# ignacio-rocco/detectorch

Hardware: AMD Instinct MI355X
Metric: images/sec Mask R-CNN R-50-FPN 1333x800 (region-proposal hot path) (higher is better)
Workload: dtype f32

## Files before the change

### detectorch_amd/csrc/roi_align.hip

```cpp
#include <stdlib.h>

#include <type_traits>

#include "roi_align_common.h"

namespace dtc {

constexpr int kRoiAlignThreads = 256;
constexpr int kMaxTableEntries = 2048;

template <typename TOut>
__device__ __forceinline__ void zero_outputs(TOut* out, int n) {
  for (int o = threadIdx.x; o < n; o += kRoiAlignThreads) out[o] = from_f32<TOut>(0.f);
}

__device__ __forceinline__ void build_axis_tables(AxisEntry* tab, const RoiHead& hd, const dtc_feat_level& L, int ny, int nx,
                                                  int ymul = 1, int xmul = 1) {
  for (int t = threadIdx.x; t < ny + nx; t += kRoiAlignThreads) {
    const bool is_y = t < ny;
    const int u = is_y ? t : t - ny, g = is_y ? hd.gh : hd.gw, mul = is_y ? ymul : xmul;
    AxisEntry e = make_axis(is_y ? hd.sh : hd.sw, is_y ? hd.bin_h : hd.bin_w, u / g, u % g, g, is_y ? L.height : L.width);
    e.lo *= mul; e.hi *= mul;
    tab[t] = e;
  }
// ... 489 lines not shown
  const bool vec = full && ((L.stride_h | L.stride_w | L.stride_n) & 3) == 0 && ((c0 & 3) == 0) &&
                   (reinterpret_cast<uintptr_t>(L.data) & 15) == 0;
  if (4 * q < nc) {
    for (int bin = slot; bin < bins; bin += kRoiAlignThreads / NQ4) {
      const int ph = bin / p.pooled_w, pw = bin - ph * p.pooled_w;
      float a0 = 0.f, a1 = 0.f, a2 = 0.f, a3 = 0.f;
      if (vec && tab_ok && gh == 2 && gw == 2) {
        const AxisEntry x0e = xtab[pw * 2], x1e = xtab[pw * 2 + 1];
        const AxisEntry y0e = ytab[ph * 2], y1e = ytab[ph * 2 + 1];
        float4 t[16];
        t[0] = load4(base + y0e.lo + x0e.lo); t[1] = load4(base + y0e.lo + x0e.hi);
        t[2] = load4(base + y0e.hi + x0e.lo); t[3] = load4(base + y0e.hi + x0e.hi);
        t[4] = load4(base + y0e.lo + x1e.lo); t[5] = load4(base + y0e.lo + x1e.hi);
        t[6] = load4(base + y0e.hi + x1e.lo); t[7] = load4(base + y0e.hi + x1e.hi);
        t[8] = load4(base + y1e.lo + x0e.lo); t[9] = load4(base + y1e.lo + x0e.hi);
        t[10] = load4(base + y1e.hi + x0e.lo); t[11] = load4(base + y1e.hi + x0e.hi);
        t[12] = load4(base + y1e.lo + x1e.lo); t[13] = load4(base + y1e.lo + x1e.hi);
        t[14] = load4(base + y1e.hi + x1e.lo); t[15] = load4(base + y1e.hi + x1e.hi);
#pragma unroll
        for (int sidx = 0; sidx < 4; sidx++) {
          const AxisEntry& y = (sidx < 2) ? y0e : y1e;
          const AxisEntry& x = (sidx & 1) ? x1e : x0e;
          const float w1 = y.h * x.h, w2 = y.h * x.l, w3 = y.l * x.h, w4 = y.l * x.l;
          const float4 v1 = t[sidx * 4], v2 = t[sidx * 4 + 1], v3 = t[sidx * 4 + 2], v4 = t[sidx * 4 + 3];
          a0 += w1 * v1.x + w2 * v2.x + w3 * v3.x + w4 * v4.x;
          a1 += w1 * v1.y + w2 * v2.y + w3 * v3.y + w4 * v4.y;
          a2 += w1 * v1.z + w2 * v2.z + w3 * v3.z + w4 * v4.z;
          a3 += w1 * v1.w + w2 * v2.w + w3 * v3.w + w4 * v4.w;
        }
      } else {
      for (int iy = 0; iy < gh; iy++) {
        const AxisEntry y = tab_ok ? ytab[ph * gh + iy] : [&] { AxisEntry e = make_axis(sh, bin_h, ph, iy, gh, L.height); e.lo *= (int)L.stride_h; e.hi *= (int)L.stride_h; return e; }();
        for (int ix = 0; ix < gw; ix++) {
          const AxisEntry x = tab_ok ? xtab[pw * gw + ix] : [&] { AxisEntry e = make_axis(sw, bin_w, pw, ix, gw, L.width); e.lo *= (int)L.stride_w; e.hi *= (int)L.stride_w; return e; }();
          const float w1 = y.h * x.h, w2 = y.h * x.l, w3 = y.l * x.h, w4 = y.l * x.l;
          float4 v1, v2, v3, v4;
          if (vec) {
            v1 = load4(base + y.lo + x.lo); v2 = load4(base + y.lo + x.hi);
            v3 = load4(base + y.hi + x.lo); v4 = load4(base + y.hi + x.hi);
          } else {
            const TIn* t1 = base + y.lo + x.lo; const TIn* t2 = base + y.lo + x.hi;
            const TIn* t3 = base + y.hi + x.lo; const TIn* t4 = base + y.hi + x.hi;
            const int nv = nc - 4 * q;
            v1 = make_float4(to_f32<TIn>(t1[0]), nv > 1 ? to_f32<TIn>(t1[1]) : 0.f, nv > 2 ? to_f32<TIn>(t1[2]) : 0.f, nv > 3 ? to_f32<TIn>(t1[3]) : 0.f);
            v2 = make_float4(to_f32<TIn>(t2[0]), nv > 1 ? to_f32<TIn>(t2[1]) : 0.f, nv > 2 ? to_f32<TIn>(t2[2]) : 0.f, nv > 3 ? to_f32<TIn>(t2[3]) : 0.f);
            v3 = make_float4(to_f32<TIn>(t3[0]), nv > 1 ? to_f32<TIn>(t3[1]) : 0.f, nv > 2 ? to_f32<TIn>(t3[2]) : 0.f, nv > 3 ? to_f32<TIn>(t3[3]) : 0.f);
            v4 = make_float4(to_f32<TIn>(t4[0]), nv > 1 ? to_f32<TIn>(t4[1]) : 0.f, nv > 2 ? to_f32<TIn>(t4[2]) : 0.f, nv > 3 ? to_f32<TIn>(t4[3]) : 0.f);
          }
          a0 += w1 * v1.x + w2 * v2.x + w3 * v3.x + w4 * v4.x;
          a1 += w1 * v1.y + w2 * v2.y + w3 * v3.y + w4 * v4.y;
          a2 += w1 * v1.z + w2 * v2.z + w3 * v3.z + w4 * v4.z;
          a3 += w1 * v1.w + w2 * v2.w + w3 * v3.w + w4 * v4.w;
        }
      }
      }
      float* so = slab + (4 * q) * bins + bin;
      if (inv_count != 0.f) { so[0] = a0 * inv_count; so[bins] = a1 * inv_count; so[2 * bins] = a2 * inv_count; so[3 * bins] = a3 * inv_count; }
      else { so[0] = fdiv(a0, count); so[bins] = fdiv(a1, count); so[2 * bins] = fdiv(a2, count); so[3 * bins] = fdiv(a3, count); }
    }
  }
  __syncthreads();
  store_slab_vec<TOut, kRoiAlignThreads>(out, slab, nc * bins, tid);
}

const RoiAlignKnobs& roi_align_knobs() {
  static const RoiAlignKnobs knobs = [] {
    RoiAlignKnobs k;
    const auto first_not_0 = [](const char* name, bool dflt) { const char* e = getenv(name); return e ? e[0] != '0' : dflt; };
    const auto is_set = [](const char* name) { return getenv(name) != nullptr; };
    const auto number = [](const char* name, int dflt) { const char* e = getenv(name); return e ? atoi(e) : dflt; };
    const auto in_range = [&](const char* name, int lo, int hi, int dflt) { const int v = number(name, dflt); return v >= lo && v <= hi ? v : dflt; };
    k.tile = first_not_0("DTC_ROIALIGN_TILE", true);
    k.map = first_not_0("DTC_ROIALIGN_MAP", true);
    k.general = is_set("DTC_ROIALIGN_GENERAL");
    k.nhwc_direct = !is_set("DTC_ROIALIGN_NO_NHWC_DIRECT");
    k.nhwc16 = first_not_0("DTC_RA_NHWC16", true);
    k.nhwc_direct32 = first_not_0("DTC_RA_NHWC_DIRECT32", true);
    k.xcd = !is_set("DTC_RA_NO_XCD");
    k.cts64 = !is_set("DTC_RA_NO_CTS64");
    const int cb = number("DTC_RA_TILE_CHBLOCK", 0);
    if (cb >= 4 && (cb & 3) == 0) k.tile_ch_block = cb;
    k.tile_cb_major = number("DTC_RA_TILE_CBMAJOR", 1) != 0;
    k.tile_lds16_kb = in_range("DTC_RA_TILE_LDS16_KB", 36, 156, 0);
    k.map_prep = number("DTC_RA_MAP_PREP", 1) != 0;
    k.map_pitch = first_not_0("DTC_RA_MAP_PITCH", true);
    k.nhwc_lds = number("DTC_RA_NHWC_LDS", 1) != 0;
    k.nhwc_lds_kb = in_range("DTC_RA_NHWC_LDS_KB", 24, 160, 0);
    k.nhwc_pipe = in_range("DTC_RA_NHWC_PIPE", 0, 2, 1);
    k.nhwc_pipe16 = number("DTC_RA_NHWC_PIPE16", 0) != 0;
    k.nhwc_lds_16bit = number("DTC_RA_NHWC_LDS_16BIT", 0) != 0;
    return k;
  }();
  return knobs;
}

constexpr int kLdsKernelBytes = 52 * 1024;

template <typename TIn, typename TOut, int CB>
static int launch_nhwc_cb(const RoiAlignParams& p, hipStream_t stream) {
  const size_t smem = (size_t)kLdsTableFloats * 4 + (size_t)CB * p.pooled_h * p.pooled_w * 4 + 16;
  if (raise_lds_once<roi_align_fwd_nhwc<TIn, TOut, CB>>(160 * 1024) != DTC_OK) return DTC_ELAUNCH;
  const int nct = ceil_div(p.channels, CB);
  hipLaunchKernelGGL((roi_align_fwd_nhwc<TIn, TOut, CB>), dim3((unsigned)p.n_rois * nct), dim3(kRoiAlignThreads), smem, stream, p);
  DTC_CHECK_LAUNCH();
  return DTC_OK;
}

template <typename TIn, typename TOut>
static int launch_nhwc(const RoiAlignParams& p, hipStream_t stream) {
  if (p.n_rois == 0) return DTC_OK;
  if constexpr (sizeof(TIn) == 2) {
    if (p.pooled_h * p.pooled_w > 64 && p.channels % 32 == 0) return launch_nhwc_cb<TIn, TOut, 32>(p, stream);
  }
  return launch_nhwc_cb<TIn, TOut, 64>(p, stream);
}

template <typename TIn, typename TOut>
static int launch_lds(const RoiAlignParams& p, hipStream_t stream) {
  if (p.n_rois == 0) return DTC_OK;
  if (raise_lds_once<roi_align_fwd_lds<TIn, TOut>>(160 * 1024) != DTC_OK) return DTC_ELAUNCH;
  const int nct = ceil_div(p.channels, p.ch_block);
  hipLaunchKernelGGL((roi_align_fwd_lds<TIn, TOut>), dim3((unsigned)p.n_rois * nct), dim3(kRoiAlignThreads), kLdsKernelBytes, stream, p,
                     kLdsKernelBytes / 4);
  DTC_CHECK_LAUNCH();
  return DTC_OK;
}

template <typename TIn, typename TOut>
static int launch_general(const RoiAlignParams& p, hipStream_t stream) {
  if (p.n_rois == 0) return DTC_OK;
  int entries = p.sampling_ratio > 0 ? (p.pooled_h + p.pooled_w) * p.sampling_ratio : kMaxTableEntries;
  if (entries > kMaxTableEntries) entries = kMaxTableEntries;
  size_t smem = (size_t)entries * sizeof(AxisEntry);
  dim3 grid(p.n_rois, ceil_div(p.channels, p.ch_tile));
  hipLaunchKernelGGL((roi_align_fwd_general<TIn, TOut>), grid, dim3(kRoiAlignThreads), smem, stream, p);
  DTC_CHECK_LAUNCH();
  return DTC_OK;
}

enum { kKernNhwc, kKernLds, kKernGeneral };
static int launch_typed(int kind, const RoiAlignParams& p, int in_dtype, int out_dtype, hipStream_t s) {
  return dispatch_io_pair(in_dtype, out_dtype, [&](auto tin, auto tout) {
    typedef tag_type<decltype(tin)> TIn;
    typedef tag_type<decltype(tout)> TOut;
    return kind == kKernNhwc ? launch_nhwc<TIn, TOut>(p, s) : kind == kKernLds ? launch_lds<TIn, TOut>(p, s) : launch_general<TIn, TOut>(p, s);
  });
}

}

static int roi_align_dispatch(const dtc_feat_level* levels, int n_levels, int channels, int in_dtype, const float* rois,
                             int roi_cols, const int32_t* roi_levels, const int32_t* roi_order, const float* roi_desc,
                             int n_rois, int pooled_h, int pooled_w, int sampling_ratio, void* out, int out_dtype,
                             dtc_stream_t stream, void* workspace = nullptr, size_t workspace_bytes = 0) {
  if (!levels || n_levels < 1 || n_levels > DTC_MAX_LEVELS || channels < 1 || n_rois < 0 || pooled_h < 1 ||
      pooled_w < 1 || (roi_cols != 4 && roi_cols != 5) || (n_rois > 0 && ((!rois && !roi_desc) || !out)))
    return DTC_EINVAL;
  const dtc::RoiAlignKnobs& cfg = dtc::roi_align_knobs();
  dtc::RoiAlignParams p;
  for (int i = 0; i < n_levels; i++) {
    if (!levels[i].data || levels[i].height < 1 || levels[i].width < 1) return DTC_EINVAL;
    p.lv[i] = levels[i];
  }
  p.rois = rois; p.roi_levels = roi_levels; p.roi_order = roi_order; p.roi_desc = roi_desc; p.out = out;
  p.n_levels = n_levels; p.channels = channels; p.roi_cols = roi_cols; p.n_rois = n_rois;
  p.pooled_h = pooled_h; p.pooled_w = pooled_w; p.sampling_ratio = sampling_ratio;
// ... 73 lines not shown
```

### detectorch_amd/csrc/roi_align_common.h

```cpp
#pragma once
#include "dtc_common.h"

namespace dtc {

struct RoiAlignParams {
  dtc_feat_level lv[DTC_MAX_LEVELS];
  const float* rois;
  const int32_t* roi_levels;
  const int32_t* roi_order;
  const float* roi_desc;
  void* out;
  int n_levels, channels, roi_cols, n_rois, pooled_h, pooled_w, sampling_ratio, ch_tile;
  int ch_block;
  int cts64;
  int xcd_remap;
  const void* prep = nullptr;
};

constexpr int kXcds = 8;
__device__ __forceinline__ int xcd_work_item(int b, int n, int enabled) {
  if (!enabled || n < 2 * kXcds) return b;
  const int x = b % kXcds, j = b / kXcds;
  const int q = n / kXcds, r = n - q * kXcds;
  return x * q + min(x, r) + j;
// ... 44 lines not shown
    w.d0 = make_float4(b, roi[0], roi[1], roi[2]);
    w.d1 = make_float4(roi[3], (float)lvl, (float)r, 0.f);
  }
  return w;
}

__device__ __forceinline__ RoiHead roi_head_from_raw(const RoiAlignParams& p, const RoiRaw& w) {
  RoiHead h;
  h.b = (int)w.d0.x; h.lvl = (int)w.d1.y; h.r = (int)w.d1.z;
  const float x1 = w.d0.y, y1 = w.d0.z, x2 = w.d0.w, y2 = w.d1.x;
  h.sw = h.sh = 0.f; h.rw = h.rh = 1.f; h.bin_h = h.bin_w = 1.f; h.gh = h.gw = 1; h.count = 1.f; h.inv_count = 1.f;
  if (h.lvl < 0 || h.lvl >= p.n_levels) return h;
  const float s = p.lv[h.lvl].spatial_scale;
  h.sw = x1 * s; h.sh = y1 * s;
  const float ew = x2 * s, eh = y2 * s;
  h.rw = fmaxf(ew - h.sw, 1.f); h.rh = fmaxf(eh - h.sh, 1.f);
  h.bin_h = fdiv(h.rh, (float)p.pooled_h); h.bin_w = fdiv(h.rw, (float)p.pooled_w);
  h.gh = p.sampling_ratio > 0 ? p.sampling_ratio : (int)ceilf(fdiv(h.rh, (float)p.pooled_h));
  h.gw = p.sampling_ratio > 0 ? p.sampling_ratio : (int)ceilf(fdiv(h.rw, (float)p.pooled_w));
  const int gg = h.gh * h.gw;
  h.count = (float)gg;
  h.inv_count = ((gg & (gg - 1)) == 0) ? fdiv(1.f, h.count) : 0.f;
  return h;
}

__device__ __forceinline__ RoiHead load_roi_head(const RoiAlignParams& p, int ri) {
  return roi_head_from_raw(p, load_roi_raw(p, ri));
}

template <typename T> __device__ __forceinline__ f32x2 mul_pair16(uint32_t u, float w);
template <> __device__ __forceinline__ f32x2 mul_pair16<__half>(uint32_t u, float w) {
  f32x2 r;
  asm("v_fma_mix_f32 %0, %2, %3, %4 op_sel:[0,0,0] op_sel_hi:[1,0,0]\n\tv_fma_mix_f32 %1, %2, %3, %4 op_sel:[1,0,0] op_sel_hi:[1,0,0]"
      : "=&v"(r.x), "=&v"(r.y) : "v"(u), "v"(w), "s"(-0.0f));
  return r;
}
template <> __device__ __forceinline__ f32x2 mul_pair16<bf16_t>(uint32_t u, float w) {
  const f32x2 v = {__uint_as_float(u << 16), __uint_as_float(u & 0xffff0000u)};
  return v * w;
}
template <> __device__ __forceinline__ f32x2 mul_pair16<float>(uint32_t, float) { return f32x2{0.f, 0.f}; }

template <typename T> __device__ __forceinline__ void fma_pair16(f32x2& acc, uint32_t u, float w);
template <> __device__ __forceinline__ void fma_pair16<__half>(f32x2& acc, uint32_t u, float w) {
  asm("v_fma_mix_f32 %0, %2, %3, %0 op_sel:[0,0,0] op_sel_hi:[1,0,0]\n\tv_fma_mix_f32 %1, %2, %3, %1 op_sel:[1,0,0] op_sel_hi:[1,0,0]"
      : "+v"(acc.x), "+v"(acc.y) : "v"(u), "v"(w));
}
template <> __device__ __forceinline__ void fma_pair16<bf16_t>(f32x2& acc, uint32_t u, float w) {
  const f32x2 v = {__uint_as_float(u << 16), __uint_as_float(u & 0xffff0000u)};
  const f32x2 w2 = {w, w};
  acc = __builtin_elementwise_fma(v, w2, acc);
}
template <> __device__ __forceinline__ void fma_pair16<float>(f32x2&, uint32_t, float) {}

template <typename T> struct dtype_tag { typedef T type; };
template <typename Tag> using tag_type = typename Tag::type;
template <typename F>
inline int dispatch_io_pair(int in_dtype, int out_dtype, F&& f) {
  if (in_dtype == DTC_F32 && out_dtype == DTC_F32) return f(dtype_tag<float>{}, dtype_tag<float>{});
  if (in_dtype == DTC_F16 && out_dtype == DTC_F32) return f(dtype_tag<__half>{}, dtype_tag<float>{});
  if (in_dtype == DTC_F16 && out_dtype == DTC_F16) return f(dtype_tag<__half>{}, dtype_tag<__half>{});
  if (in_dtype == DTC_F32 && out_dtype == DTC_F16) return f(dtype_tag<float>{}, dtype_tag<__half>{});
  if (in_dtype == DTC_BF16 && out_dtype == DTC_F32) return f(dtype_tag<bf16_t>{}, dtype_tag<float>{});
  if (in_dtype == DTC_BF16 && out_dtype == DTC_BF16) return f(dtype_tag<bf16_t>{}, dtype_tag<bf16_t>{});
  if (in_dtype == DTC_F32 && out_dtype == DTC_BF16) return f(dtype_tag<float>{}, dtype_tag<bf16_t>{});
  return DTC_EUNSUPPORTED;
}
inline bool io_pair_supported(int in_dtype, int out_dtype) {
  return dispatch_io_pair(in_dtype, out_dtype, [](auto, auto) { return (int)DTC_OK; }) == DTC_OK;
}

struct RoiAlignKnobs {
  bool tile = true;
  bool map = true;
  bool general = false;
  bool nhwc_direct = true;
  bool nhwc16 = true;
  bool nhwc_direct32 = true;
  bool xcd = true;
  bool cts64 = true;
  int tile_ch_block = 0;
  int tile_cb_major = 1;
  int tile_lds16_kb = 0;
  bool map_prep = true;
  bool map_pitch = true;
  int nhwc_lds = 1;
  int nhwc_lds_kb = 0;
  int nhwc_pipe = 1;
  int nhwc_pipe16 = 0;
  bool nhwc_lds_16bit = false;
};
const RoiAlignKnobs& roi_align_knobs();

bool roi_align_tile_supported(const RoiAlignParams& p, int in_dtype, int out_dtype);
int launch_roi_align_tile(const RoiAlignParams& p, int in_dtype, int out_dtype, hipStream_t stream);
bool roi_align_map_supported(const RoiAlignParams& p, int in_dtype, int out_dtype);
int launch_roi_align_map(const RoiAlignParams& p, int in_dtype, int out_dtype, hipStream_t stream);
void roi_align_set_exact(int exact);
int roi_align_get_exact();
size_t roi_align_map_workspace_bytes(int n_rois);
int launch_roi_align_map_ws(const RoiAlignParams& p, int in_dtype, int out_dtype, void* workspace, size_t workspace_bytes, hipStream_t stream);

bool roi_align_nhwc_lds_supported(const RoiAlignParams& p, int in_dtype, int out_dtype);
int launch_roi_align_nhwc_lds(const RoiAlignParams& p, int in_dtype, int out_dtype, hipStream_t stream);

bool roi_align_nhwc16_supported(const RoiAlignParams& p, int in_dtype, int out_dtype);
int launch_roi_align_nhwc16(const RoiAlignParams& p, int in_dtype, int out_dtype, hipStream_t stream);

}
```

### detectorch_amd/csrc/roi_align_tile.hip

```cpp

#include <type_traits>

#include "roi_align_common.h"

namespace dtc {

constexpr int kTileMaxK = 32;
constexpr int kTileRoiBytes = 48, kTileGroupBytes = 32;
constexpr int kTileHdrBytes = kTileMaxK * (kTileRoiBytes + kTileGroupBytes) + 16;
template <int NT> struct TileShape;
template <> struct TileShape<256> { static constexpr int kUnits = 8, kWaves = 3, kLdsKB = 52, kWaves16 = 4, kLds16KB = 38; };

struct TileRoi {
  int lvl, b, x0, x1, y0, y1, r, valid;
  float sh, sw, bin_h, bin_w;
};
static_assert(sizeof(TileRoi) == kTileRoiBytes, "TileRoi layout");
struct TileGroup { int first, count, kind, x0, x1, y0, y1, pad; };
enum { kGrpPool = 0, kGrpZero = 1, kGrpAbsent = 2, kGrpGather = 3 };

__device__ __forceinline__ __amdgpu_buffer_rsrc_t make_srd(const void* base) {
  return __builtin_amdgcn_make_buffer_rsrc(const_cast<void*>(base), 0, 0xffffffff, 0x00020000);
}
template <typename TIn> struct Piece4;
template <> struct Piece4<float> {
  typedef float4 Raw;
  static __device__ __forceinline__ Raw raw(__amdgpu_buffer_rsrc_t r, uint32_t voff, uint32_t soff) { return ld(r, voff, soff); }
  static __device__ __forceinline__ float4 ld(__amdgpu_buffer_rsrc_t r, uint32_t voff, uint32_t soff) {
    const u32x4 v = __builtin_amdgcn_raw_buffer_load_b128(r, voff, soff, 0);
    return make_float4(__uint_as_float(v.x), __uint_as_float(v.y), __uint_as_float(v.z), __uint_as_float(v.w));
  }
};
template <> struct Piece4<__half> {
  typedef u32x2 Raw;
  static __device__ __forceinline__ Raw raw(__amdgpu_buffer_rsrc_t r, uint32_t voff, uint32_t soff) { return __builtin_amdgcn_raw_buffer_load_b64(r, voff, soff, 0); }
  static __device__ __forceinline__ float4 ld(__amdgpu_buffer_rsrc_t r, uint32_t voff, uint32_t soff) {
    const u32x2 v = __builtin_amdgcn_raw_buffer_load_b64(r, voff, soff, 0);
    const uint32_t x = v.x, y = v.y;
    const __half2 a = *reinterpret_cast<const __half2*>(&x), b = *reinterpret_cast<const __half2*>(&y);
    return make_float4(__low2float(a), __high2float(a), __low2float(b), __high2float(b));
  }
};
template <> struct Piece4<bf16_t> {
  typedef u32x2 Raw;
  static __device__ __forceinline__ Raw raw(__amdgpu_buffer_rsrc_t r, uint32_t voff, uint32_t soff) { return __builtin_amdgcn_raw_buffer_load_b64(r, voff, soff, 0); }
  static __device__ __forceinline__ float4 ld(__amdgpu_buffer_rsrc_t r, uint32_t voff, uint32_t soff) {
    const u32x2 v = __builtin_amdgcn_raw_buffer_load_b64(r, voff, soff, 0);
    return bf16x4_to_f32(make_uint2(v.x, v.y));
  }
};

__device__ __forceinline__ int uni(int v) { return __builtin_amdgcn_readfirstlane(v); }

#ifdef DTC_TILE_TRACE
constexpr int kTraceSlots = 16;
__device__ unsigned long long g_tile_trace[kTraceSlots * 16384];
struct TileTrace {
  unsigned long long last, acc[kTraceSlots];
  __device__ __forceinline__ void start() { for (int i = 0; i < kTraceSlots; i++) acc[i] = 0; last = __builtin_readcyclecounter(); }
  __device__ __forceinline__ void mark(int i) { const unsigned long long n = __builtin_readcyclecounter(); acc[i] += n - last; last = n; }
};
#define TT_MARK(i) tt.mark(i)
#else
struct TileTrace {};
#define TT_MARK(i) ((void)0)
#endif

template <typename TIn> struct TileLds { typedef float T; static constexpr int kSlot = 16, kShift = 4; };
template <> struct TileLds<__half> { typedef uint16_t T; static constexpr int kSlot = 8, kShift = 3; };
template <> struct TileLds<bf16_t> { typedef uint16_t T; static constexpr int kSlot = 8, kShift = 3; };

template <typename TIn, int NT> struct TileBounds { static constexpr int kWaves = TileShape<NT>::kWaves; };
template <int NT> struct TileBounds<__half, NT> { static constexpr int kWaves = TileShape<NT>::kWaves16; };
template <int NT> struct TileBounds<bf16_t, NT> { static constexpr int kWaves = TileShape<NT>::kWaves16; };

__device__ __forceinline__ int tile_phys(int px) { return px + (px >> 3); }

struct TileItem {
  int a[2][2][4];
  float yl[2], yh[2], xl[2], xh[2];
  bool on;
};

template <typename TOut> __device__ __forceinline__ void store_quad(TOut* d, float4 v);
template <> __device__ __forceinline__ void store_quad<float>(float* d, float4 v) { store_stream16(d, v); }
template <> __device__ __forceinline__ void store_quad<__half>(__half* d, float4 v) {
  const __half2 a = __floats2half2_rn(v.x, v.y), b = __floats2half2_rn(v.z, v.w);
  store_stream8(d, *reinterpret_cast<const uint32_t*>(&a), *reinterpret_cast<const uint32_t*>(&b));
}
template <> __device__ __forceinline__ void store_quad<bf16_t>(bf16_t* d, float4 v) {
  store_stream8(d, (uint32_t)from_f32<bf16_t>(v.x).bits | ((uint32_t)from_f32<bf16_t>(v.y).bits << 16),
                (uint32_t)from_f32<bf16_t>(v.z).bits | ((uint32_t)from_f32<bf16_t>(v.w).bits << 16));
}

enum { kStageScalar = 0, kStageVec = 1, kStageVecUnaligned = 2 };

struct TileGeom {
  int first, count;
  int y0, x0a, ngx, npos;
  int plane;
  int nq_pass;
  int mode;
};

template <typename TIn, typename TOut, int NT, bool FUSED>
__device__ __forceinline__ void tile_passes(const RoiAlignParams& p, const dtc_feat_level& L, const TIn* fbase, int c0, int nc,
                                            int bins, float* slab, typename TileLds<TIn>::T* win, const TileRoi* troi, const TileGeom& g,
                                            const TileItem& it, int rl, int bin, TileTrace& tt) {
  constexpr int NW = NT / 64;
  constexpr int U = TileShape<NT>::kUnits;
  typedef typename TileLds<TIn>::T TL;
  constexpr bool L16 = sizeof(TL) == 2;
  constexpr int SB = TileLds<TIn>::kSlot;
  const int tid = threadIdx.x, lane = tid & 63, wv = tid >> 6, pl = lane & 15, cl = (lane >> 4) & 3;
  const int npos = g.npos, ngx = g.ngx, plane = g.plane, nq_pass = g.nq_pass;
  const int nchunk = (npos + 15) >> 4;
  const int KC = ceil_div(nchunk, NW);
  const float rinv = 1.0f / (float)ngx;
  const int nq_tot = ceil_div(nc, 4);
  const bool vec = g.mode != kStageScalar;
  uint32_t uoff[U];
  int ulds[U];
  const int nu = KC * nq_pass;
  if (vec) {
    const int sh32 = (int)L.stride_h, sc32 = (int)L.stride_c;
    int q = 0, i = 0;
#pragma unroll
    for (int u = 0; u < U; u++) {
      const bool dup = u >= nu;
      const int pos = min((wv + (dup ? 0 : i) * NW) * 16 + pl, npos - 1);
      const int row = (int)(((float)pos + 0.5f) * rinv);
      const int gx = pos - row * ngx;
      const int qq = dup ? 0 : q;
      int col = g.x0a + 4 * gx, sft = 0;
      if (g.mode == kStageVecUnaligned) { sft = max(0, col + 3 - (L.width - 1)); col -= sft; }
      uoff[u] = ((uint32_t)((g.y0 + row) * sh32 + col + (4 * qq + cl) * sc32) * (uint32_t)sizeof(TIn)) | ((uint32_t)sft << 30);
      ulds[u] = qq * plane * 4 + ((4 * pos + (pos >> 1)) << 2) + cl;
      if (++i == KC) { i = 0; q++; }
    }
  }
  const __amdgpu_buffer_rsrc_t srd = make_srd(fbase);
  const uint32_t pass_bytes = (uint32_t)(L.stride_c * (int64_t)sizeof(TIn));
  typename Piece4<TIn>::Raw v[U];
  auto issue = [&](int cs) {
    const uint32_t soff = (uint32_t)cs * pass_bytes;
    if (g.mode == kStageVec) {
#pragma unroll
      for (int u = 0; u < U; u++) v[u] = Piece4<TIn>::raw(srd, uoff[u], soff);
    } else {
#pragma unroll
      for (int u = 0; u < U; u++) v[u] = Piece4<TIn>::raw(srd, uoff[u] & 0x3fffffffu, soff);
    }
  };
  auto commit_as = [&](auto shifted_tag) {
    constexpr bool SHIFTED = decltype(shifted_tag)::value;
    if constexpr (SHIFTED) asm volatile("" ::: "memory");
#pragma unroll
    for (int u = 0; u < U; u++) {
      if constexpr (L16) {
        uint32_t w0 = v[u].x & 0xffffu, w1 = v[u].x >> 16, w2 = v[u].y & 0xffffu, w3 = v[u].y >> 16;
        if constexpr (SHIFTED) {
          const uint32_t sft = uoff[u] >> 30;
          w0 = sft == 0 ? w0 : sft == 1 ? w1 : sft == 2 ? w2 : w3;
          w1 = sft == 0 ? w1 : sft == 1 ? w2 : w3;
          w2 = sft == 0 ? w2 : w3;
        }
        TL* d = win + ulds[u];
        d[0] = (TL)w0; d[4] = (TL)w1; d[8] = (TL)w2; d[12] = (TL)w3;
      } else {
        float4 w = v[u];
        if constexpr (SHIFTED) {
          const uint32_t sft = uoff[u] >> 30;
          w.x = sft == 0 ? w.x : sft == 1 ? w.y : sft == 2 ? w.z : w.w;
          w.y = sft == 0 ? w.y : sft == 1 ? w.z : w.w;
          w.z = sft == 0 ? w.z : w.w;
        }
        TL* d = win + ulds[u];
        d[0] = w.x; d[4] = w.y; d[8] = w.z; d[12] = w.w;
      }
    }
  };
  auto commit = [&]() {
    if (g.mode == kStageVecUnaligned) commit_as(std::true_type{}); else commit_as(std::false_type{});
  };
  auto lds_val = [&](const TIn& x) -> TL {
    if constexpr (L16) return *reinterpret_cast<const uint16_t*>(&x); else return to_f32<TIn>(x);
  };
  auto stage_scalar = [&](int cs) {
#pragma unroll 1
    for (int q = 0; q < nq_pass; q++) {
      const int cq = cs + 4 * q;
      if (cq >= nc) break;
      const int cle = min(cl, nc - 1 - cq);
      const TIn* base = fbase + (int64_t)(cq + cle) * L.stride_c;
#pragma unroll 1
      for (int t = wv; t < nchunk; t += NW) {
        const int pos = min(t * 16 + pl, npos - 1);
        const int row = (int)(((float)pos + 0.5f) * rinv);
        const int gx = pos - row * ngx;
        const int rem = L.width - 1 - (g.x0a + 4 * gx);
        const TIn* s = base + (int64_t)(g.y0 + row) * L.stride_h + (int64_t)(g.x0a + 4 * gx) * L.stride_w;
        TL* d = win + q * plane * 4 + ((4 * pos + (pos >> 1)) << 2) + cl;
        d[0] = lds_val(s[0]);
        d[4] = lds_val(s[(int64_t)min(1, rem) * L.stride_w]);
        d[8] = lds_val(s[(int64_t)min(2, rem) * L.stride_w]);
        d[12] = lds_val(s[(int64_t)min(3, rem) * L.stride_w]);
      }
    }
  };
  const bool quad_ok = ((p.channels | c0) & 3) == 0;
  auto store_slab = [&](int cs, int nq) {
    const int nch = min(4 * nq, nc - cs);
    TOut* out = reinterpret_cast<TOut*>(p.out);
    if (quad_ok && nch == 4 * nq) {
      const int n4 = nq * bins, total = g.count * n4;
      const float r4 = 1.0f / (float)n4;
      const int cs_off = cs * bins;
      for (int idx = tid; idx < total; idx += NT) {
        const int k = (int)(((float)idx + 0.5f) * r4);
        const int e = idx - __mul24(k, n4);
        const float4 val = reinterpret_cast<const float4*>(slab)[idx];
        const uint64_t ob = *reinterpret_cast<const uint64_t*>(&troi[g.first + k].x0);
        store_quad<TOut>(out + (ob + (uint64_t)(uint32_t)(cs_off + 4 * e)), val);
      }
    } else {
      const int per = nch * bins, total = g.count * per;
      for (int idx = tid; idx < total; idx += NT) {
        const int k = idx / per, e = idx - k * per;
        out[((size_t)troi[g.first + k].r * p.channels + c0 + cs) * bins + e] = from_f32<TOut>(slab[k * 4 * nq * bins + e]);
      }
    }
  };

#ifdef DTC_TILE_REPLAY
  {
    uint32_t sink = 0;
    if (DTC_TILE_REPLAY == 1 || DTC_TILE_REPLAY == 4) { if (vec) issue(0); }
    int cs_prev = 0, nq_prev = 0;
#pragma unroll 1
    for (int qs = 0; qs < nq_tot; qs += nq_pass) {
      const int cs = 4 * qs;
      const int nq_cur = min(nq_pass, nq_tot - qs);
      if (DTC_TILE_REPLAY == 1) {
#pragma unroll
        for (int u = 0; u < U; u++) { if constexpr (L16) sink ^= v[u].x ^ v[u].y; else sink ^= __float_as_uint(v[u].x) ^ __float_as_uint(v[u].w); }
        if (vec && qs + nq_pass < nq_tot) issue(cs + 4 * nq_pass);
      } else if (DTC_TILE_REPLAY == 4) {
        if (vec) commit(); else stage_scalar(cs);
        __syncthreads();
        if (vec && qs + nq_pass < nq_tot) issue(cs + 4 * nq_pass);
        __syncthreads();
      } else if (DTC_TILE_REPLAY == 2) {
        store_slab(cs, nq_cur);
      } else if (DTC_TILE_REPLAY == 3) {
        __syncthreads();
        if (it.on) {
          float* so = slab + rl * (4 * nq_cur * bins) + bin;
#pragma unroll 1
          for (int q = 0; q < nq_cur; q++) {
            const char* wq = reinterpret_cast<const char*>(win) + uni(q * plane * SB);
            f32x2 a01 = {0.f, 0.f}, a23 = {0.f, 0.f};
#pragma unroll
            for (int iy = 0; iy < 2; iy++) {
              if constexpr (!L16) {
                f32x4 t[2][4];
#pragma unroll
                for (int ix = 0; ix < 2; ix++)
#pragma unroll
                  for (int k = 0; k < 4; k++) t[ix][k] = *reinterpret_cast<const f32x4*>(__builtin_assume_aligned(wq + it.a[iy][ix][k], 16));
#pragma unroll
                for (int ix = 0; ix < 2; ix++) {
                  const float w1 = it.yh[iy] * it.xh[ix], w2 = it.yh[iy] * it.xl[ix], w3 = it.yl[iy] * it.xh[ix], w4 = it.yl[iy] * it.xl[ix];
                  a01 += w1 * t[ix][0].lo + w2 * t[ix][1].lo + w3 * t[ix][2].lo + w4 * t[ix][3].lo;
                  a23 += w1 * t[ix][0].hi + w2 * t[ix][1].hi + w3 * t[ix][2].hi + w4 * t[ix][3].hi;
                }
              }
              __builtin_amdgcn_sched_barrier(0);
            }
            float* o = so + uni(4 * q * bins);
            o[0] = a01.x * 0.25f; o[bins] = a01.y * 0.25f; o[2 * bins] = a23.x * 0.25f; o[3 * bins] = a23.y * 0.25f;
          }
        }
        __syncthreads();
      }
      cs_prev = cs; nq_prev = nq_cur;
    }
    (void)cs_prev; (void)nq_prev;
    if (sink == 0x9e3779b9u && p.n_rois < 0) reinterpret_cast<uint32_t*>(p.out)[0] = sink;
  }
  TT_MARK(10);
}
#else
  TT_MARK(3);
  if (vec) issue(0);
  int cs_prev = 0, nq_prev = 0;
#pragma unroll 1
  for (int qs = 0; qs < nq_tot; qs += nq_pass) {
    const int cs = 4 * qs;
    const int nq_cur = min(nq_pass, nq_tot - qs);
    if (vec) commit(); else stage_scalar(cs);
    TT_MARK(4);
    if (nq_prev) store_slab(cs_prev, nq_prev);
    TT_MARK(5);
    __syncthreads();
    TT_MARK(6);
    if (vec && qs + nq_pass < nq_tot) issue(cs + 4 * nq_pass);
    TT_MARK(7);
    if (it.on) {
      float* so = slab + rl * (4 * nq_cur * bins) + bin;
#pragma unroll 1
      for (int q = 0; q < nq_cur; q++) {
        const char* wq = reinterpret_cast<const char*>(win) + uni(q * plane * SB);
        f32x2 a01 = {0.f, 0.f}, a23 = {0.f, 0.f};
#pragma unroll
        for (int iy = 0; iy < 2; iy++) {
          if constexpr (L16 && FUSED) {
            u32x2 t[2][4];
#pragma unroll
            for (int ix = 0; ix < 2; ix++)
#pragma unroll
              for (int k = 0; k < 4; k++)
                t[ix][k] = *reinterpret_cast<const u32x2*>(__builtin_assume_aligned(wq + it.a[iy][ix][k], 8));
#pragma unroll
            for (int ix = 0; ix < 2; ix++) {
              const float w1 = it.yh[iy] * it.xh[ix], w2 = it.yh[iy] * it.xl[ix];
              const float w3 = it.yl[iy] * it.xh[ix], w4 = it.yl[iy] * it.xl[ix];
              fma_pair16<TIn>(a01, t[ix][0].x, w1); fma_pair16<TIn>(a23, t[ix][0].y, w1);
              fma_pair16<TIn>(a01, t[ix][1].x, w2); fma_pair16<TIn>(a23, t[ix][1].y, w2);
              fma_pair16<TIn>(a01, t[ix][2].x, w3); fma_pair16<TIn>(a23, t[ix][2].y, w3);
              fma_pair16<TIn>(a01, t[ix][3].x, w4); fma_pair16<TIn>(a23, t[ix][3].y, w4);
            }
          } else if constexpr (L16) {
            u32x2 t[2][4];
#pragma unroll
            for (int ix = 0; ix < 2; ix++)
#pragma unroll
              for (int k = 0; k < 4; k++)
                t[ix][k] = *reinterpret_cast<const u32x2*>(__builtin_assume_aligned(wq + it.a[iy][ix][k], 8));
#pragma unroll
            for (int ix = 0; ix < 2; ix++) {
              const float w1 = it.yh[iy] * it.xh[ix], w2 = it.yh[iy] * it.xl[ix];
              const float w3 = it.yl[iy] * it.xh[ix], w4 = it.yl[iy] * it.xl[ix];
              f32x2 s01 = mul_pair16<TIn>(t[ix][0].x, w1) + mul_pair16<TIn>(t[ix][1].x, w2);
              s01 = s01 + mul_pair16<TIn>(t[ix][2].x, w3);
              s01 = s01 + mul_pair16<TIn>(t[ix][3].x, w4);
              f32x2 s23 = mul_pair16<TIn>(t[ix][0].y, w1) + mul_pair16<TIn>(t[ix][1].y, w2);
              s23 = s23 + mul_pair16<TIn>(t[ix][2].y, w3);
              s23 = s23 + mul_pair16<TIn>(t[ix][3].y, w4);
              a01 = a01 + s01; a23 = a23 + s23;
            }
          } else {
            f32x4 t[2][4];
#pragma unroll
            for (int ix = 0; ix < 2; ix++)
#pragma unroll
              for (int k = 0; k < 4; k++)
                t[ix][k] = *reinterpret_cast<const f32x4*>(__builtin_assume_aligned(wq + it.a[iy][ix][k], 16));
#pragma unroll
            for (int ix = 0; ix < 2; ix++) {
              const float w1 = it.yh[iy] * it.xh[ix], w2 = it.yh[iy] * it.xl[ix];
              const float w3 = it.yl[iy] * it.xh[ix], w4 = it.yl[iy] * it.xl[ix];
              a01 += w1 * t[ix][0].lo + w2 * t[ix][1].lo + w3 * t[ix][2].lo + w4 * t[ix][3].lo;
              a23 += w1 * t[ix][0].hi + w2 * t[ix][1].hi + w3 * t[ix][2].hi + w4 * t[ix][3].hi;
            }
          }
          __builtin_amdgcn_sched_barrier(0);
        }
        float* o = so + uni(4 * q * bins);
        const float a0 = a01.x, a1 = a01.y, a2 = a23.x, a3 = a23.y;
        o[0] = a0 * 0.25f; o[bins] = a1 * 0.25f; o[2 * bins] = a2 * 0.25f; o[3 * bins] = a3 * 0.25f;
      }
    }
    TT_MARK(8);
    __syncthreads();
    TT_MARK(9);
    cs_prev = cs; nq_prev = nq_cur;
  }
  if (nq_prev) store_slab(cs_prev, nq_prev);
  TT_MARK(10);
}
#endif


__device__ __forceinline__ int tile_work_item(int b, int n, int reverse) {
  if (n < 2 * kXcds || (reverse & 2)) return (reverse & 1) ? n - 1 - b : b;
  const int x = b % kXcds, j = b / kXcds;
  const int q = n / kXcds, r = n - q * kXcds;
  const int start = x * q + min(x, r), qx = q + (x < r ? 1 : 0);
  return start + ((reverse & 1) ? qx - 1 - j : j);
}

template <typename TIn, typename TOut, int NT, bool FUSED>
__global__ __launch_bounds__(NT, (TileBounds<TIn, NT>::kWaves)) void roi_align_fwd_tile(RoiAlignParams p, int kgroup, int lds_bytes, int nq_cap, int merge_pct, int reverse) {
  extern __shared__ __attribute__((aligned(16))) unsigned char smem[];
  TileRoi* troi = reinterpret_cast<TileRoi*>(smem);
  TileGroup* tgrp = reinterpret_cast<TileGroup*>(smem + kTileMaxK * kTileRoiBytes);
  int* ngp = reinterpret_cast<int*>(smem + kTileMaxK * (kTileRoiBytes + kTileGroupBytes));
  const int slab_bytes = kgroup * p.pooled_h * p.pooled_w * 16 * nq_cap;
  float* slab = reinterpret_cast<float*>(smem + kTileHdrBytes);
  typedef typename TileLds<TIn>::T TL;
  constexpr int SB = TileLds<TIn>::kSlot;
  TL* win = reinterpret_cast<TL*>(smem + kTileHdrBytes + slab_bytes);
  const int win_bytes = lds_bytes - kTileHdrBytes - slab_bytes;
  constexpr int NW = NT / 64;
  constexpr int kMaxPos = TileShape<NT>::kUnits * NW * 16;
  const int tid = threadIdx.x;
  const int nct = ceil_div(p.channels, p.ch_block);
  int wi = tile_work_item(blockIdx.x, gridDim.x, reverse);
  int grp = wi / nct;
  int c0 = (wi - grp * nct) * p.ch_block;
  {
    const int ngrp = (int)gridDim.x / nct;
    if ((reverse & 4) && ngrp % kXcds == 0 && ngrp >= 2 * kXcds) {
      const int x = blockIdx.x % kXcds, j = blockIdx.x / kXcds, ngx = ngrp / kXcds;
      const int cbi = j / ngx, gl = j - cbi * ngx;
      grp = x * ngx + ((reverse & 1) ? ngx - 1 - gl : gl);
      c0 = cbi * p.ch_block;
      wi = grp * nct + cbi;
    }
  }
  const int nc = min(p.ch_block, p.channels - c0);
  const int bins = p.pooled_h * p.pooled_w;
  const int K = kgroup;
  TileTrace tt;
#ifdef DTC_TILE_TRACE
  tt.start();
  const unsigned long long wall0 = __builtin_amdgcn_s_memrealtime();
#endif

  if (tid < 64) {
    TileRoi t;
    t.lvl = -1; t.b = 0; t.x0 = t.x1 = t.y0 = t.y1 = 0; t.r = 0; t.valid = 0; t.sh = t.sw = 0.f; t.bin_h = t.bin_w = 1.f;
    const int ri = grp * K + tid;
    if (tid < K && ri < p.n_rois) {
      const RoiHead hd = load_roi_head(p, ri);
      t.valid = 1; t.r = hd.r; t.b = hd.b; t.sh = hd.sh; t.sw = hd.sw; t.bin_h = hd.bin_h; t.bin_w = hd.bin_w;
      if (hd.lvl >= 0 && hd.lvl < p.n_levels) {
        t.lvl = hd.lvl;
        const int H = p.lv[hd.lvl].height, W = p.lv[hd.lvl].width;
        t.y0 = make_axis(hd.sh, hd.bin_h, 0, 0, 2, H).lo;
        t.y1 = make_axis(hd.sh, hd.bin_h, p.pooled_h - 1, 1, 2, H).hi;
        t.x0 = make_axis(hd.sw, hd.bin_w, 0, 0, 2, W).lo;
        t.x1 = make_axis(hd.sw, hd.bin_w, p.pooled_w - 1, 1, 2, W).hi;
      }
    }
    if (tid < K) {
      troi[tid] = t;
      *reinterpret_cast<uint64_t*>(&troi[tid].x0) = ((uint64_t)(uint32_t)t.r * (uint64_t)p.channels + (uint64_t)c0) * (uint64_t)(p.pooled_h * p.pooled_w);
    }
    auto bc = [](int v, int k) { return __builtin_amdgcn_readlane(v, k); };
    int ng = 0, k = 0;
    while (k < K) {
      const int ks = uni(k);
      const int a_lvl = bc(t.lvl, ks), a_b = bc(t.b, ks), a_valid = bc(t.valid, ks);
      const int a_x0 = bc(t.x0, ks), a_x1 = bc(t.x1, ks), a_y0 = bc(t.y0, ks), a_y1 = bc(t.y1, ks);
      TileGroup g;
      g.first = k; g.count = 1; g.x0 = a_x0; g.x1 = a_x1; g.y0 = a_y0; g.y1 = a_y1; g.pad = 0;
      if (!a_valid) g.kind = kGrpAbsent;
      else if (a_lvl < 0) g.kind = kGrpZero;
      else {
        const int ngx0 = (a_x1 >> 2) - (a_x0 >> 2) + 1, th0 = a_y1 - a_y0 + 1, npos0 = th0 * ngx0;
        if (npos0 > kMaxPos || (4 * npos0 + (npos0 >> 1) + 1) * SB > win_bytes || bins > NT) {
          g.kind = kGrpGather;
        } else {
          g.kind = kGrpPool;
          long long sum_px = (long long)th0 * (a_x1 - a_x0 + 1);
          while (k + g.count < K && (g.count + 1) * bins <= NT) {
            const int js = uni(k + g.count);
            const int n_lvl = bc(t.lvl, js), n_b = bc(t.b, js), n_valid = bc(t.valid, js);
            if (!n_valid || n_lvl != a_lvl || n_b != a_b) break;
            const int n_x0 = bc(t.x0, js), n_x1 = bc(t.x1, js), n_y0 = bc(t.y0, js), n_y1 = bc(t.y1, js);
            const int ux0 = min(g.x0, n_x0), ux1 = max(g.x1, n_x1), uy0 = min(g.y0, n_y0), uy1 = max(g.y1, n_y1);
            const int ungx = (ux1 >> 2) - (ux0 >> 2) + 1, uth = uy1 - uy0 + 1, unpos = uth * ungx;
            if (unpos > kMaxPos || (4 * unpos + (unpos >> 1) + 1) * SB > win_bytes) break;
            const long long n_px = (long long)(n_y1 - n_y0 + 1) * (n_x1 - n_x0 + 1);
            const long long u_px = (long long)uth * (ux1 - ux0 + 1);
            if (u_px * 100 > (sum_px + n_px) * merge_pct) break;
            g.x0 = ux0; g.x1 = ux1; g.y0 = uy0; g.y1 = uy1; g.count++;
            sum_px += n_px;
          }
        }
      }
      if (tid == 0) tgrp[ng] = g;
      ng++;
      k += g.count;
    }
    if (tid == 0) *ngp = ng;
  }
  __syncthreads();
  TT_MARK(0);
  TT_MARK(1);

  const int ngroups = uni(*ngp);
  for (int gi = 0; gi < ngroups; gi++) {
    const int first = uni(tgrp[gi].first), count = uni(tgrp[gi].count), kind = uni(tgrp[gi].kind);
    if (kind == kGrpAbsent) continue;
    if (kind == kGrpZero) {
      TOut* oz = reinterpret_cast<TOut*>(p.out) + ((size_t)uni(troi[first].r) * p.channels + c0) * bins;
      for (int o = tid; o < nc * bins; o += NT) oz[o] = from_f32<TOut>(0.f);
      continue;
    }
    const int lvl = uni(troi[first].lvl), b = uni(troi[first].b);
    const dtc_feat_level L = p.lv[lvl];
    const TIn* fbase = reinterpret_cast<const TIn*>(L.data) + (int64_t)b * L.stride_n + (int64_t)c0 * L.stride_c;
    if (kind == kGrpGather) {
      const RoiHead hd = load_roi_head(p, grp * K + first);
      TOut* og = reinterpret_cast<TOut*>(p.out) + ((size_t)hd.r * p.channels + c0) * bins;
      for (int o = tid; o < nc * bins; o += NT) {
        const int c = o / bins, bin = o - c * bins;
        const int ph = bin / p.pooled_w, pw = bin - ph * p.pooled_w;
        const TIn* d = fbase + (int64_t)c * L.stride_c;
        float acc = 0.f;
        for (int iy = 0; iy < 2; iy++) {
          const AxisEntry y = make_axis(hd.sh, hd.bin_h, ph, iy, 2, L.height);
          const int64_t ylo = (int64_t)y.lo * L.stride_h, yhi = (int64_t)y.hi * L.stride_h;
          for (int ix = 0; ix < 2; ix++) {
            const AxisEntry x = make_axis(hd.sw, hd.bin_w, pw, ix, 2, L.width);
            const int64_t xlo = (int64_t)x.lo * L.stride_w, xhi = (int64_t)x.hi * L.stride_w;
            const float w1 = y.h * x.h, w2 = y.h * x.l, w3 = y.l * x.h, w4 = y.l * x.l;
            acc += w1 * to_f32<TIn>(d[ylo + xlo]) + w2 * to_f32<TIn>(d[ylo + xhi]) + w3 * to_f32<TIn>(d[yhi + xlo]) +
                   w4 * to_f32<TIn>(d[yhi + xhi]);
          }
        }
        og[o] = from_f32<TOut>(acc * 0.25f);
      }
      continue;
    }
    const int gx0 = uni(tgrp[gi].x0), gx1 = uni(tgrp[gi].x1), gy0 = uni(tgrp[gi].y0), gy1 = uni(tgrp[gi].y1);
    TileGeom g;
    g.first = first; g.count = count;
    g.y0 = gy0; g.x0a = gx0 & ~3;
    g.ngx = (gx1 >> 2) - (gx0 >> 2) + 1;
    const int tw = 4 * g.ngx, th = gy1 - gy0 + 1;
    g.npos = th * g.ngx;
    g.plane = 4 * g.npos + (g.npos >> 1) + 1;
    const int esz = (int)sizeof(TIn);
    const bool lin = L.stride_w == 1 && ((nc | c0) & 3) == 0 && L.stride_h > 0 && L.stride_c > 0 &&
                     L.stride_h * L.height + L.stride_c * 4 * TileShape<NT>::kUnits < (1ll << 26);
    const bool al16 = ((L.width | L.stride_h | L.stride_c | L.stride_n) & 3) == 0 &&
                      (reinterpret_cast<uintptr_t>(L.data) & (4 * sizeof(TIn) - 1)) == 0;
    const bool al4 = L.width >= 4 && (((L.width | L.stride_h | L.stride_c | L.stride_n) * esz) & 3) == 0 &&
                     (reinterpret_cast<uintptr_t>(L.data) & 3) == 0;
    g.mode = !lin ? kStageScalar : al16 ? kStageVec : al4 ? kStageVecUnaligned : kStageScalar;
    const int KC = ceil_div((g.npos + 15) >> 4, NW);
    g.nq_pass = max(1, min(min(win_bytes / (g.plane * SB), TileShape<NT>::kUnits / KC), min(ceil_div(nc, 4), nq_cap)));
    while (ceil_div(nc, 4) % g.nq_pass) g.nq_pass--;
    const int n_it = count * bins;
    TileItem it;
    it.on = tid < n_it;
    const int itx = it.on ? tid : 0;
    const int rl = itx / bins, bin = itx - rl * bins;
    const int ph = bin / p.pooled_w, pw = bin - ph * p.pooled_w;
    const TileRoi hd = troi[first + rl];
    int ylo[2], yhi[2], xlo[2], xhi[2];
#pragma unroll
    for (int i = 0; i < 2; i++) {
      const AxisEntry ey = make_axis(hd.sh, hd.bin_h, ph, i, 2, L.height);
      const AxisEntry ex = make_axis(hd.sw, hd.bin_w, pw, i, 2, L.width);
      it.yl[i] = ey.l; it.yh[i] = ey.h; it.xl[i] = ex.l; it.xh[i] = ex.h;
      ylo[i] = (ey.lo - gy0) * tw; yhi[i] = (ey.hi - gy0) * tw;
      xlo[i] = ex.lo - g.x0a; xhi[i] = ex.hi - g.x0a;
    }
#pragma unroll
    for (int iy = 0; iy < 2; iy++)
#pragma unroll
      for (int ix = 0; ix < 2; ix++) {
        constexpr int SS = TileLds<TIn>::kShift;
        int t0 = tile_phys(ylo[iy] + xlo[ix]) << SS, t1 = tile_phys(ylo[iy] + xhi[ix]) << SS;
        int t2 = tile_phys(yhi[iy] + xlo[ix]) << SS, t3 = tile_phys(yhi[iy] + xhi[ix]) << SS;
        asm volatile("" : "+v"(t0), "+v"(t1), "+v"(t2), "+v"(t3));
        it.a[iy][ix][0] = t0; it.a[iy][ix][1] = t1; it.a[iy][ix][2] = t2; it.a[iy][ix][3] = t3;
      }
    TT_MARK(2);
    tile_passes<TIn, TOut, NT, FUSED>(p, L, fbase, c0, nc, bins, slab, win, troi, g, it, rl, bin, tt);
  }
#ifdef DTC_TILE_TRACE
  if (tid == 0 && blockIdx.x < 16384) {
    unsigned long long* o = g_tile_trace + (size_t)blockIdx.x * kTraceSlots;
    for (int i = 0; i < 11; i++) o[i] = tt.acc[i];
    o[11] = wall0; o[12] = __builtin_amdgcn_s_memrealtime();
    o[13] = (unsigned long long)ngroups; o[14] = (unsigned long long)__builtin_amdgcn_s_getreg((4 << 0) | (0 << 6) | (31 << 11));
    o[15] = (unsigned long long)wi;
  }
#endif
}

#ifdef DTC_TILE_TRACE
}
extern "C" __attribute__((visibility("default"))) int dtc_debug_tile_trace(void* host_dst, size_t bytes) {
  return hipMemcpyFromSymbol(host_dst, HIP_SYMBOL(dtc::g_tile_trace), bytes, 0, hipMemcpyDeviceToHost) == hipSuccess ? 0 : -1;
}
namespace dtc {
#endif

constexpr int kTileThreads = 256;
constexpr int kTileMergePct = 250;
constexpr int kTileNqCap = 4;
constexpr int kTileReverse = 1;

template <typename TIn, typename TOut, int NT, bool FUSED>
static int launch_tile_nt(RoiAlignParams p, hipStream_t stream) {
  const RoiAlignKnobs& cfg = roi_align_knobs();
  const int bins = p.pooled_h * p.pooled_w;
  int K = NT / bins;
  K = K < 1 ? 1 : (K > kTileMaxK ? kTileMaxK : K);
  if (K * bins > NT) K = NT / bins;
  if (K < 1) return DTC_EUNSUPPORTED;
  const int lds_b = (sizeof(TIn) == 2 ? (cfg.tile_lds16_kb ? cfg.tile_lds16_kb : TileShape<NT>::kLds16KB) : TileShape<NT>::kLdsKB) * 1024;
  if (raise_lds_once<roi_align_fwd_tile<TIn, TOut, NT, FUSED>>(160 * 1024) != DTC_OK) return DTC_ELAUNCH;
  const int nq_cap = kTileNqCap;
  if (kTileHdrBytes + K * bins * 16 * nq_cap + 20 * 1024 > lds_b) return DTC_EUNSUPPORTED;
  const int ngrp = ceil_div(p.n_rois, K);
  int cb = cfg.tile_ch_block ? cfg.tile_ch_block : ((long long)ngrp * ceil_div(p.channels, 128) >= 6144 ? 128 : 64);
  while (!cfg.tile_ch_block && cb > 32 && (long long)ngrp * ceil_div(p.channels, cb) < 2048) cb >>= 1;
  p.ch_block = cb;
  const int nct = ceil_div(p.channels, p.ch_block);
  hipLaunchKernelGGL((roi_align_fwd_tile<TIn, TOut, NT, FUSED>), dim3((unsigned)ngrp * nct), dim3(NT), lds_b, stream, p, K, lds_b, nq_cap, kTileMergePct, (kTileReverse ? 1 : 0) | (p.xcd_remap ? 0 : 2) | (cfg.tile_cb_major ? 4 : 0));
  DTC_CHECK_LAUNCH();
  return DTC_OK;
}

template <typename TIn, typename TOut>
static int launch_tile_t(const RoiAlignParams& p, hipStream_t stream) {
  if constexpr (sizeof(TIn) == 2) { if (!roi_align_get_exact()) return launch_tile_nt<TIn, TOut, kTileThreads, true>(p, stream); }
  return launch_tile_nt<TIn, TOut, kTileThreads, false>(p, stream);
}

bool roi_align_tile_supported(const RoiAlignParams& p, int in_dtype, int out_dtype) {
  if (p.sampling_ratio != 2) return false;
  if (p.pooled_h * p.pooled_w > kTileThreads) return false;
  return io_pair_supported(in_dtype, out_dtype);
}

int launch_roi_align_tile(const RoiAlignParams& p, int in_dtype, int out_dtype, hipStream_t stream) {
  if (p.n_rois == 0) return DTC_OK;
  return dispatch_io_pair(in_dtype, out_dtype, [&](auto tin, auto tout) {
    return launch_tile_t<tag_type<decltype(tin)>, tag_type<decltype(tout)>>(p, stream);
  });
}

}
```

Baseline: 14340.

## Store ROIAlign tile results directly from registers via DPP quad transpose

Adds a register-store path for the tiled ROIAlign kernel. Lanes exchange their four per-channel results with a DPP quad transpose, then write them straight to global memory as 4-wide stores. This skips the LDS slab and its separate store_slab pass, and frees that LDS for a larger feature window. It only applies when one ROI fills the block (K==1), the bin count is a multiple of 4, and channel offsets are 4-aligned. Writes are now spread across the compute loop and may coalesce less well than the slab copy.

```diff
diff --git a/detectorch_amd/csrc/roi_align.hip b/detectorch_amd/csrc/roi_align.hip
--- a/detectorch_amd/csrc/roi_align.hip
+++ b/detectorch_amd/csrc/roi_align.hip
@@ -595,6 +595,7 @@
     if (cb >= 4 && (cb & 3) == 0) k.tile_ch_block = cb;
     k.tile_cb_major = number("DTC_RA_TILE_CBMAJOR", 1) != 0;
     k.tile_lds16_kb = in_range("DTC_RA_TILE_LDS16_KB", 36, 156, 0);
+    k.tile_regstore = first_not_0("DTC_RA_TILE_REGSTORE", true);
     k.map_prep = number("DTC_RA_MAP_PREP", 1) != 0;
     k.map_pitch = first_not_0("DTC_RA_MAP_PITCH", true);
     k.nhwc_lds = number("DTC_RA_NHWC_LDS", 1) != 0;
diff --git a/detectorch_amd/csrc/roi_align_common.h b/detectorch_amd/csrc/roi_align_common.h
--- a/detectorch_amd/csrc/roi_align_common.h
+++ b/detectorch_amd/csrc/roi_align_common.h
@@ -150,6 +150,7 @@
   int tile_ch_block = 0;
   int tile_cb_major = 1;
   int tile_lds16_kb = 0;
+  bool tile_regstore = true;
   bool map_prep = true;
   bool map_pitch = true;
   int nhwc_lds = 1;
diff --git a/detectorch_amd/csrc/roi_align_tile.hip b/detectorch_amd/csrc/roi_align_tile.hip
--- a/detectorch_amd/csrc/roi_align_tile.hip
+++ b/detectorch_amd/csrc/roi_align_tile.hip
@@ -93,6 +93,16 @@
                 (uint32_t)from_f32<bf16_t>(v.z).bits | ((uint32_t)from_f32<bf16_t>(v.w).bits << 16));
 }
 
+__device__ __forceinline__ float quad_xor1(float x) { return __uint_as_float((uint32_t)__builtin_amdgcn_update_dpp(0, (int)__float_as_uint(x), 0xB1, 0xf, 0xf, false)); }
+__device__ __forceinline__ float quad_xor2(float x) { return __uint_as_float((uint32_t)__builtin_amdgcn_update_dpp(0, (int)__float_as_uint(x), 0x4E, 0xf, 0xf, false)); }
+__device__ __forceinline__ void quad_transpose(float& r0, float& r1, float& r2, float& r3, int lane) {
+  const bool b0 = lane & 1, b1 = lane & 2;
+  const float t01 = quad_xor1(b0 ? r0 : r1), t23 = quad_xor1(b0 ? r2 : r3);
+  r0 = b0 ? t01 : r0; r1 = b0 ? r1 : t01; r2 = b0 ? t23 : r2; r3 = b0 ? r3 : t23;
+  const float t02 = quad_xor2(b1 ? r0 : r2), t13 = quad_xor2(b1 ? r1 : r3);
+  r0 = b1 ? t02 : r0; r2 = b1 ? r2 : t02; r1 = b1 ? t13 : r1; r3 = b1 ? r3 : t13;
+}
+
 enum { kStageScalar = 0, kStageVec = 1, kStageVecUnaligned = 2 };
 
 struct TileGeom {
@@ -106,7 +116,7 @@
 template <typename TIn, typename TOut, int NT, bool FUSED>
 __device__ __forceinline__ void tile_passes(const RoiAlignParams& p, const dtc_feat_level& L, const TIn* fbase, int c0, int nc,
                                             int bins, float* slab, typename TileLds<TIn>::T* win, const TileRoi* troi, const TileGeom& g,
-                                            const TileItem& it, int rl, int bin, TileTrace& tt) {
+                                            const TileItem& it, int rl, int bin, bool regstore, TileTrace& tt) {
   constexpr int NW = NT / 64;
   constexpr int U = TileShape<NT>::kUnits;
   typedef typename TileLds<TIn>::T TL;
@@ -231,6 +241,8 @@
       }
     }
   };
+  TOut* oreg = reinterpret_cast<TOut*>(p.out);
+  if (regstore) oreg += *reinterpret_cast<const uint64_t*>(&troi[g.first].x0) + (uint64_t)(uint32_t)((bin & 3) * bins + (bin & ~3));
 
 #ifdef DTC_TILE_REPLAY
   {
@@ -300,7 +312,7 @@
     const int nq_cur = min(nq_pass, nq_tot - qs);
     if (vec) commit(); else stage_scalar(cs);
     TT_MARK(4);
-    if (nq_prev) store_slab(cs_prev, nq_prev);
+    if (nq_prev && !regstore) store_slab(cs_prev, nq_prev);
     TT_MARK(5);
     __syncthreads();
     TT_MARK(6);
@@ -308,6 +320,7 @@
     TT_MARK(7);
     if (it.on) {
       float* so = slab + rl * (4 * nq_cur * bins) + bin;
+      TOut* oq = oreg + uni(cs * bins);
 #pragma unroll 1
       for (int q = 0; q < nq_cur; q++) {
         const char* wq = reinterpret_cast<const char*>(win) + uni(q * plane * SB);
@@ -366,9 +379,14 @@
           }
           __builtin_amdgcn_sched_barrier(0);
         }
-        float* o = so + uni(4 * q * bins);
-        const float a0 = a01.x, a1 = a01.y, a2 = a23.x, a3 = a23.y;
-        o[0] = a0 * 0.25f; o[bins] = a1 * 0.25f; o[2 * bins] = a2 * 0.25f; o[3 * bins] = a3 * 0.25f;
+        float a0 = a01.x * 0.25f, a1 = a01.y * 0.25f, a2 = a23.x * 0.25f, a3 = a23.y * 0.25f;
+        if (regstore) {
+          quad_transpose(a0, a1, a2, a3, tid);
+          store_quad<TOut>(oq + uni(4 * q * bins), make_float4(a0, a1, a2, a3));
+        } else {
+          float* o = so + uni(4 * q * bins);
+          o[0] = a0; o[bins] = a1; o[2 * bins] = a2; o[3 * bins] = a3;
+        }
       }
     }
     TT_MARK(8);
@@ -376,7 +394,7 @@
     TT_MARK(9);
     cs_prev = cs; nq_prev = nq_cur;
   }
-  if (nq_prev) store_slab(cs_prev, nq_prev);
+  if (nq_prev && !regstore) store_slab(cs_prev, nq_prev);
   TT_MARK(10);
 }
 #endif
@@ -396,12 +414,8 @@
   TileRoi* troi = reinterpret_cast<TileRoi*>(smem);
   TileGroup* tgrp = reinterpret_cast<TileGroup*>(smem + kTileMaxK * kTileRoiBytes);
   int* ngp = reinterpret_cast<int*>(smem + kTileMaxK * (kTileRoiBytes + kTileGroupBytes));
-  const int slab_bytes = kgroup * p.pooled_h * p.pooled_w * 16 * nq_cap;
-  float* slab = reinterpret_cast<float*>(smem + kTileHdrBytes);
   typedef typename TileLds<TIn>::T TL;
   constexpr int SB = TileLds<TIn>::kSlot;
-  TL* win = reinterpret_cast<TL*>(smem + kTileHdrBytes + slab_bytes);
-  const int win_bytes = lds_bytes - kTileHdrBytes - slab_bytes;
   constexpr int NW = NT / 64;
   constexpr int kMaxPos = TileShape<NT>::kUnits * NW * 16;
   const int tid = threadIdx.x;
@@ -422,6 +436,16 @@
   const int nc = min(p.ch_block, p.channels - c0);
   const int bins = p.pooled_h * p.pooled_w;
   const int K = kgroup;
+#ifdef DTC_TILE_REPLAY
+  const bool regstore = false;
+#else
+  const bool regstore = (reverse & 8) && ((p.channels | c0 | nc) & 3) == 0;
+#endif
+  const int slab_bytes = regstore ? 0 : kgroup * bins * 16 * nq_cap;
+  const int nq_lim = regstore ? TileShape<NT>::kUnits : nq_cap;
+  float* slab = reinterpret_cast<float*>(smem + kTileHdrBytes);
+  TL* win = reinterpret_cast<TL*>(smem + kTileHdrBytes + slab_bytes);
+  const int win_bytes = lds_bytes - kTileHdrBytes - slab_bytes;
   TileTrace tt;
 #ifdef DTC_TILE_TRACE
   tt.start();
@@ -543,7 +567,7 @@
                      (reinterpret_cast<uintptr_t>(L.data) & 3) == 0;
     g.mode = !lin ? kStageScalar : al16 ? kStageVec : al4 ? kStageVecUnaligned : kStageScalar;
     const int KC = ceil_div((g.npos + 15) >> 4, NW);
-    g.nq_pass = max(1, min(min(win_bytes / (g.plane * SB), TileShape<NT>::kUnits / KC), min(ceil_div(nc, 4), nq_cap)));
+    g.nq_pass = max(1, min(min(win_bytes / (g.plane * SB), TileShape<NT>::kUnits / KC), min(ceil_div(nc, 4), nq_lim)));
     while (ceil_div(nc, 4) % g.nq_pass) g.nq_pass--;
     const int n_it = count * bins;
     TileItem it;
@@ -572,7 +596,7 @@
         it.a[iy][ix][0] = t0; it.a[iy][ix][1] = t1; it.a[iy][ix][2] = t2; it.a[iy][ix][3] = t3;
       }
     TT_MARK(2);
-    tile_passes<TIn, TOut, NT, FUSED>(p, L, fbase, c0, nc, bins, slab, win, troi, g, it, rl, bin, tt);
+    tile_passes<TIn, TOut, NT, FUSED>(p, L, fbase, c0, nc, bins, slab, win, troi, g, it, rl, bin, regstore, tt);
   }
 #ifdef DTC_TILE_TRACE
   if (tid == 0 && blockIdx.x < 16384) {
@@ -615,7 +639,8 @@
   while (!cfg.tile_ch_block && cb > 32 && (long long)ngrp * ceil_div(p.channels, cb) < 2048) cb >>= 1;
   p.ch_block = cb;
   const int nct = ceil_div(p.channels, p.ch_block);
-  hipLaunchKernelGGL((roi_align_fwd_tile<TIn, TOut, NT, FUSED>), dim3((unsigned)ngrp * nct), dim3(NT), lds_b, stream, p, K, lds_b, nq_cap, kTileMergePct, (kTileReverse ? 1 : 0) | (p.xcd_remap ? 0 : 2) | (cfg.tile_cb_major ? 4 : 0));
+  const bool regstore = cfg.tile_regstore && K == 1 && bins % 4 == 0;
+  hipLaunchKernelGGL((roi_align_fwd_tile<TIn, TOut, NT, FUSED>), dim3((unsigned)ngrp * nct), dim3(NT), lds_b, stream, p, K, lds_b, nq_cap, kTileMergePct, (kTileReverse ? 1 : 0) | (p.xcd_remap ? 0 : 2) | (cfg.tile_cb_major ? 4 : 0) | (regstore ? 8 : 0));
   DTC_CHECK_LAUNCH();
   return DTC_OK;
 }
```

Result: slower. 13950 (-2.7%).
